# DassHydro-dev/smash

Measured on AMD Instinct MI355X. Metric: cell-timesteps/s, forward+adjoint sweep, higher is better.
Workload: dtype f32

## Files before the change

smash_amd/csrc/smashx.hip:

```cpp
#include "../../include/smashx.h"

#include <hip/hip_runtime.h>
#include <rccl/rccl.h>

#include <dlfcn.h>

#include <algorithm>
#include <functional>
#include <numeric>
#include <cstdio>
#include <cstdlib>
#include <cstring>
#include <string>
#include <vector>

#include "sx_cost.h"
#include "sx_jreg.h"
#include "sx_kernels.h"
#include "sx_ensemble.h"
#include "sx_resident.h"
#include "sx_fields.h"
#include "sx_interception.h"
#include "sx_meanforcing.h"
#include "sx_prcpindices.h"
// ... 1090 lines not shown
                        hipStream_t st, bool* ok) {
    const int h0 = p->flay.pet_hour0;
    const int d0 = (t0 + h0) / 24, d1 = (t0 + rows - 1 + h0) / 24;
    for (int r0 = 0; r0 < rows; r0 += 32768) {
        const int rr = std::min(32768, rows - r0);
        hipLaunchKernelGGL(k_encode_prcp, dim3((p->n + 255) / 256, rr), dim3(256), 0, st, p->d_prcp16 + (size_t)(t0 + r0) * p->npad,
                           d_prcp_src + (size_t)r0 * ld, idx, p->n, p->npad, ld, rr, p->flay.prcp_factor, p->d_fstatus);
    }
    hipLaunchKernelGGL(k_encode_pet, dim3((p->n + 255) / 256, d1 - d0 + 1), dim3(256), 0, st, p->d_petd, d_pet_src, idx, p->n, p->npad, ld,
                       t0, rows, h0, p->d_ratio, p->d_fstatus);
    unsigned status[2] = {0, 0};
    HIPCHK(hipMemcpyAsync(status, p->d_fstatus, sizeof(status), hipMemcpyDeviceToHost, st));
    HIPCHK(hipStreamSynchronize(st));
    HIPCHK(hipGetLastError());
    *ok = status[0] == 0;
    if (status[1]) { float g; std::memcpy(&g, &status[1], 4); p->A.prcp_gap = g; }
    p->petd_open = true;
    return 0;
}

int smashx_set_forcing_layout(smashx_plan* p, const smashx_forcing_layout* lay) {
    if (!p || !lay) return fail(SMASHX_E_ARG, "null argument");
    if (p->d_prcp || p->d_prcp16) {
        if (p->have_forcing && !p->d_prcp16 == !lay->compact) return fail(SMASHX_E_STATE, "the forcing is already resident in this layout");
        int rc = set_device(p); if (rc) return rc;
        HIPCHK(hipStreamSynchronize(p->stream)); HIPCHK(hipStreamSynchronize(p->stream_r));
        drop_compact(p);
        p->dfree(p->d_prcp); p->dfree(p->d_pet); p->d_prcp = p->d_pet = nullptr; p->A.prcp = p->A.pet = nullptr;
        p->have_forcing = false;
        p->block_seen.clear();
    }
    if (lay->compact) {
        if (p->cfg.dt != 3600.f) return fail(SMASHX_E_UNSUPPORTED, "compact forcing: the daily-PET form is defined for dt = 3600 s");
        if (!(lay->prcp_factor > 0.f) || lay->pet_hour0 < 0 || lay->pet_hour0 > 23) return fail(SMASHX_E_ARG, "bad prcp_factor / pet_hour0");
        for (int h = 0; h < 24; ++h) if (!(lay->pet_ratio[h] >= 0.f)) return fail(SMASHX_E_ARG, "pet_ratio must be >= 0");
    }
    p->flay = *lay;
    return 0;
}

int smashx_forcing_info(const smashx_plan* p, int* compact, double* bytes_per_cellstep) {
    if (!p) return fail(SMASHX_E_ARG, "null plan");
    const bool c = p->d_prcp16 != nullptr || (!p->d_prcp && p->flay.compact);
    if (compact) *compact = c ? 1 : 0;
    if (bytes_per_cellstep) *bytes_per_cellstep = c ? 2.0 + 4.0 * ((p->nt + p->flay.pet_hour0 + 23) / 24) / (double)p->nt : 8.0;
    return 0;
}

int smashx_set_forcing(smashx_plan* p, const float* prcp, const float* pet, int sparse) {
    if (!p || !prcp || !pet) return fail(SMASHX_E_ARG, "null argument");
    int rc = set_device(p); if (rc) return rc;
    if (sparse && !p->d_sparse_idx) return fail(SMASHX_E_ARG, "sparse forcing needs mesh.path at plan creation");
    const long plane = sparse ? p->n_sparse : p->n2;
    const int* idx = sparse ? p->d_sparse_idx : p->d_cell_flat;
    for (int attempt = 0; attempt < 2; ++attempt) {
        if ((rc = alloc_forcing(p))) return rc;
        const bool compact = p->d_prcp16 != nullptr;
        bool ok = true;
        if (compact) {
            const long half = std::max<long>(1, p->stage_planes / 2);
            HIPCHK(hipMemsetAsync(p->d_fstatus, 0, 2 * sizeof(unsigned), p->stream));
            HIPCHK(hipMemsetAsync(p->d_petd, 0xFF, (size_t)p->ndays * p->npad * sizeof(float), p->stream));
            for (int t = 0; t < p->nt && ok;) {
                int rows = (int)std::min<long>(half, p->nt - t);
                const int to_day_end = 24 - (t + p->flay.pet_hour0) % 24;
                if (rows > to_day_end) rows = to_day_end + (rows - to_day_end) / 24 * 24;
                float* sp = p->d_stage; float* se = p->d_stage + (size_t)half * p->n2;
                HIPCHK(hipMemcpyAsync(sp, prcp + (size_t)t * plane, (size_t)rows * plane * 4, hipMemcpyHostToDevice, p->stream));
// ... 2316 lines not shown
```

smash_amd/csrc/sx_kernels.h:

```cpp
#pragma once

#include <hip/hip_runtime.h>

#include <climits>

#include "sx_ops.h"
#include "sx_tangent.h"
#include "sx_vic.h"

#define SX_BT 4
#define SX_VBLOCK 256

__device__ __forceinline__ void sx_lds_barrier() {
    __builtin_amdgcn_fence(__ATOMIC_RELEASE, "workgroup", "local");
    __builtin_amdgcn_s_barrier();
    __builtin_amdgcn_fence(__ATOMIC_ACQUIRE, "workgroup", "local");
}

__device__ __forceinline__ void sx_lds_wave_fence() {
    __builtin_amdgcn_fence(__ATOMIC_RELEASE, "workgroup", "local");
    __builtin_amdgcn_wave_barrier();
    __builtin_amdgcn_fence(__ATOMIC_ACQUIRE, "workgroup", "local");
}

// ... 198 lines not shown
            if (i < niter && lane) {
                fifo[wpos] = v;
                const float4 o = fifo[rpos];
                wpos = wpos + 1 == depth ? 0 : wpos + 1;
                rpos = rpos + 1 == depth ? 0 : rpos + 1;
                if (GATHER) {
                    const int tb = i - d;
                    sx_gstore4(stag + (size_t)(i + smin) * A.ncs, (tb >= 0 && tb < nb) ? o : zero4);
                } else {
                    const int tb = i - spread;
                    if (plain && tb >= 0) sx_gstore4(plain + (size_t)tb * pstride, o);
                }
            }
        }
    }
}

__global__ void sx_k_prep_routing(SxDeviceArrays A) {
    SX_LIBM_INIT();
    const int k = blockIdx.x * blockDim.x + threadIdx.x;
    if (k >= A.n) return;
    const float lr = A.lr[k];
    const float f = (float)(A.flwacc[k] - 1);
    A.rt_a[k] = sx_expf(-A.dt / (lr * 60.f));
    A.rt_f[k] = f;
    A.rt_denf[k] = 0.001f * A.dx * A.dx * f;
    A.rt_denb[k] = 0.001f * (A.dx * A.dx) * f;
}

#define SX_NT 2
#ifndef SX_STILL
#define SX_STILL 1
#endif
#define SX_HIK 8
#ifndef SX_VADJ_NT
#define SX_VADJ_NT 0
#endif
template <int AUX = 0>
__device__ __forceinline__ float sx_row_load(const float* row, unsigned byte_off) {
    const __amdgpu_buffer_rsrc_t r = __builtin_amdgcn_make_buffer_rsrc((void*)row, 0, 0x7fffffff, 0x00020000);
    return __builtin_bit_cast(float, __builtin_amdgcn_raw_buffer_load_b32(r, byte_off, 0, AUX));
}
template <int AUX = 0>
__device__ __forceinline__ void sx_row_store4(float* row, unsigned byte_off, float a, float b, float c, float d) {
    typedef int sx_v4i __attribute__((ext_vector_type(4)));
    const __amdgpu_buffer_rsrc_t r = __builtin_amdgcn_make_buffer_rsrc((void*)row, 0, 0x7fffffff, 0x00020000);
    sx_v4i v = {__builtin_bit_cast(int, a), __builtin_bit_cast(int, b), __builtin_bit_cast(int, c), __builtin_bit_cast(int, d)};
    __builtin_amdgcn_raw_buffer_store_b128(v, r, byte_off, 0, AUX);
}
template <int AUX = 0>
__device__ __forceinline__ void sx_row_store(float* row, unsigned byte_off, float v) {
    const __amdgpu_buffer_rsrc_t r = __builtin_amdgcn_make_buffer_rsrc((void*)row, 0, 0x7fffffff, 0x00020000);
    __builtin_amdgcn_raw_buffer_store_b32(__builtin_bit_cast(int, v), r, byte_off, 0, AUX);
}

template <int AUX = 0>
__device__ __forceinline__ unsigned sx_row_load_u16(const unsigned short* row, unsigned byte_off) {
    const __amdgpu_buffer_rsrc_t r = __builtin_amdgcn_make_buffer_rsrc((void*)row, 0, 0x7fffffff, 0x00020000);
    return (unsigned)(unsigned short)__builtin_amdgcn_raw_buffer_load_b16(r, byte_off, 0, AUX);
}

__device__ __forceinline__ float sx_prcp_decode(const SxDeviceArrays& A, unsigned k) {
    const float v = (float)k * A.prcp_c;
    return k == 65535u ? A.prcp_gap : v;
}

typedef const __attribute__((address_space(4))) float sx_cfloat;
template <bool COMPACT>
struct SxForcing {
    const SxDeviceArrays& A;
    const unsigned kb;
    const size_t npad;
    int h;
    const char* prow; const char* erow;
    unsigned p_n, p_w; float e_n, e_w, r_n, r_w;
    __device__ __forceinline__ SxForcing(const SxDeviceArrays& A_, unsigned kb_, int t_first)
        : A(A_), kb(kb_), npad((size_t)A_.npad), h(COMPACT ? (t_first + A_.hour0) % 24 : 0),
          prow(COMPACT ? (const char*)(A_.prcp16 + (size_t)t_first * A_.npad) : (const char*)(A_.prcp + (size_t)t_first * A_.npad)),
          erow(COMPACT ? nullptr : (const char*)(A_.pet + (size_t)t_first * A_.npad)),
          p_n(0u), p_w(0u), e_n(0.f), e_w(0.f), r_n(0.f), r_w(0.f) {}
    template <int AUX, bool BACK> __device__ __forceinline__ void request(int t, bool first) {
        const long step = (long)npad * (COMPACT ? 2 : 4) * (BACK ? -1 : 1);
        if (!COMPACT) {
            p_n = __float_as_uint(sx_row_load<AUX>((const float*)prow, kb));
            e_n = sx_row_load<AUX>((const float*)erow, kb);
            prow += step; erow += step;
            return;
        }
        p_n = __float_as_uint(sx_row_load<AUX>((const float*)prow, (kb >> 1) & ~3u));
        prow += step;
        if (first || h == (BACK ? 23 : 0)) e_n = sx_row_load<AUX>(A.petd + (size_t)((t + A.hour0) / 24) * npad, kb);
        r_n = sx_row_load(A.pet_ratio + h, 0u);
        h = BACK ? (h == 0 ? 23 : h - 1) : (h == 23 ? 0 : h + 1);
    }
    __device__ __forceinline__ void hold() {
        p_w = p_n; e_w = e_n; r_w = r_n;
        sx_pinu(p_w); sx_pin1(e_w);
        if (COMPACT) sx_pin1(r_w);
    }
    __device__ __forceinline__ float prcp() const {
        if (!COMPACT) return __uint_as_float(p_w);
        return sx_prcp_decode(A, (p_w >> ((kb & 4u) << 2)) & 0xffffu);
    }
    __device__ __forceinline__ float pet() const {
        if (!COMPACT) return e_w;
        return e_w < 0.f ? e_w : e_w * r_w;
    }
};

template <bool ROW = true, class Cell>
__device__ __forceinline__ void sx_forcing_at(const SxDeviceArrays& A, int t, Cell c, float& p, float& e) {
    const size_t npad = (size_t)A.npad;
    if (A.prcp16 == nullptr) {
        if (ROW) { p = sx_row_load(A.prcp + (size_t)t * npad, c); e = sx_row_load(A.pet + (size_t)t * npad, c); }
        else { p = A.prcp[(size_t)t * npad + c]; e = A.pet[(size_t)t * npad + c]; }
        return;
    }
    p = sx_prcp_decode(A, ROW ? sx_row_load_u16(A.prcp16 + (size_t)t * npad, c >> 1) : (unsigned)A.prcp16[(size_t)t * npad + c]);
    const int q = t + A.hour0;
    const float D = ROW ? sx_row_load(A.petd + (size_t)(q / 24) * npad, c) : A.petd[(size_t)(q / 24) * npad + c];
    e = D < 0.f ? D : D * (ROW ? ((sx_cfloat*)A.pet_ratio)[q % 24] : A.pet_ratio[q % 24]);
}

#ifndef SX_VFWD_WAVES
#define SX_VFWD_WAVES 8
#endif
template <int ST, bool TAPE, bool CF>
#ifndef SX_VFWD_WAVES_GRC
#define SX_VFWD_WAVES_GRC 7
#endif
__global__ __launch_bounds__(SX_VBLOCK, (ST == 2 && CF) ? SX_VFWD_WAVES : (ST == 3 && TAPE && CF) ? SX_VFWD_WAVES_GRC : 1)
void sx_k_vert_fwd(SxDeviceArrays A, int t0, int T) {
    SX_LIBM_INIT();
    const int k = A.k0 + blockIdx.x * SX_VBLOCK + threadIdx.x;
    if (k >= A.k1) return;
    const size_t npad = (size_t)A.npad;

    const SxPlanCell<> cell{A, k};
    SxCellParams P;
    float hi = 0.f, hp = 0.f, hft = 0.f, hst = 0.f;
    sx_cell_params<ST>(cell, P);
    sx_fwd_powers<ST>(P);
    sx_levels_in<ST>(cell, hi, hp, hft, hst);

    const unsigned kb = (unsigned)k * 4u;
    SxForcing<CF> F(A, kb, t0);
    if (T > 0) F.template request<SX_NT, false>(t0, true);
    for (int tq = 0; tq * 4 < T; ++tq) {
        float q[4] = {0.f, 0.f, 0.f, 0.f};
#pragma unroll
        for (int i = 0; i < 4; ++i) {
            const int tt = tq * 4 + i;
            if (tt < T) {
                F.hold();
                if (tt + 1 < T) F.template request<SX_NT, false>(t0 + tt + 1, false);
                const float prcp = F.prcp(), pet = F.pet();
                if (TAPE) {
                    const size_t o = (size_t)tt * npad;
                    if (ST == 2 || ST == 3) {
                        if (A.tape_hi) sx_row_store<SX_NT>(A.tape_hi + o, kb, hi);
                        else if ((tt % SX_HIK) == 0) sx_row_store<SX_NT>(A.ckpt_hi + (size_t)(tt / SX_HIK) * npad, kb, hi);
                    }
                    sx_row_store<SX_NT>(A.tape_hp + o, kb, hp);
                    sx_row_store<SX_NT>(A.tape_hft + o, kb, hft);
                    if (ST == 3) sx_row_store<SX_NT>(A.tape_hst + o, kb, hst);
                }
                const bool still = SX_STILL && sx_wave_all(sx_is_still<ST>(prcp, pet, hi, hp));
                q[i] = sx_vertical_step<ST>(P, prcp, pet, hi, hp, hft, hst, still);
            }
        }
        sx_row_store4<SX_NT>(A.qtT + (size_t)tq * npad * 4, kb * 4u, q[0], q[1], q[2], q[3]);
    }
    sx_levels_out<ST>(cell, hi, hp, hft, hst);
}

__device__ __forceinline__ SxVicParams sx_vic_load(const SxDeviceArrays& A, int k) {
    return sx_vic_params(SxPlanCell<>{A, k});
}
#ifndef SX_VFWD_WAVES_VIC
#define SX_VFWD_WAVES_VIC 5
#endif
template <bool TAPE, bool CF>
__global__ __launch_bounds__(SX_VBLOCK, TAPE ? SX_VFWD_WAVES_VIC : 1) void sx_k_vert_fwd_vic(SxDeviceArrays A, int t0, int T) {
    SX_LIBM_INIT();
    const int k = A.k0 + blockIdx.x * SX_VBLOCK + threadIdx.x;
    if (k >= A.k1) return;
    const size_t npad = (size_t)A.npad;
    const SxVicParams P = sx_vic_load(A, k);
    const float cusl2_m4 = sx_pow_m4(P.cusl2);
    float husl1 = A.hi[k], husl2 = A.hp[k], hlsl = A.hft[k];
    const unsigned kb = (unsigned)k * 4u;
    SxForcing<CF> F(A, kb, t0);
    if (T > 0) F.template request<SX_NT, false>(t0, true);
    for (int tq = 0; tq * 4 < T; ++tq) {
        float q[4] = {0.f, 0.f, 0.f, 0.f};
#pragma unroll
        for (int i = 0; i < 4; ++i) {
            const int tt = tq * 4 + i;
            if (tt < T) {
                F.hold();
                if (tt + 1 < T) F.template request<SX_NT, false>(t0 + tt + 1, false);
                if (TAPE) {
                    const size_t o = (size_t)tt * npad;
                    sx_row_store<SX_NT>(A.tape_hi + o, kb, husl1);
                    sx_row_store<SX_NT>(A.tape_hp + o, kb, husl2);
                    sx_row_store<SX_NT>(A.tape_hft + o, kb, hlsl);
                }
                q[i] = sx_vic_step(P, cusl2_m4, F.prcp(), F.pet(), husl1, husl2, hlsl);
            }
        }
        sx_row_store4<SX_NT>(A.qtT + (size_t)tq * npad * 4, kb * 4u, q[0], q[1], q[2], q[3]);
    }
    A.hi[k] = husl1; A.hp[k] = husl2; A.hft[k] = hlsl;
}

#ifndef SX_VADJ_WAVES_VIC
#define SX_VADJ_WAVES_VIC 3
#endif
template <bool CF>
__global__ __launch_bounds__(SX_VBLOCK, SX_VADJ_WAVES_VIC) void sx_k_vert_adj_vic(SxDeviceArrays A, int t0, int T) {
    SX_LIBM_INIT();
    const int k = A.k0 + blockIdx.x * SX_VBLOCK + threadIdx.x;
    if (k >= A.k1) return;
    const size_t npad = (size_t)A.npad;
    const SxVicParams P = sx_vic_load(A, k);
    float cusl2_m4, cusl2_m5;
    sx_pow_m4_m5(P.cusl2, &cusl2_m4, &cusl2_m5);
    const SxPlanCell<true> grad{A, k};
    SxVicGrads G;
    sx_vic_fields_in(grad, G.b_b, G.cusl1_b, G.cusl2_b, G.clsl_b, G.ks_b, G.ds_b, G.dsm_b, G.ws_b);
    sx_vic_levels_in(grad, G.husl1_b, G.husl2_b, G.hlsl_b);
    const unsigned kb = (unsigned)k * 4u;
    SxForcing<CF> F(A, kb, t0 + T - 1);
    float n_h1 = 0.f, n_h2 = 0.f, n_hl = 0.f, n_q = 0.f;
    auto fetch = [&](int tt, bool first) {
        const size_t o = (size_t)tt * npad;
        F.template request<SX_VADJ_NT, true>(t0 + tt, first);
        n_h1 = sx_row_load<SX_VADJ_NT>(A.tape_hi + o, kb); n_h2 = sx_row_load<SX_VADJ_NT>(A.tape_hp + o, kb);
        n_hl = sx_row_load<SX_VADJ_NT>(A.tape_hft + o, kb);
        n_q = sx_row_load(A.qtT + (size_t)(tt >> 2) * npad * 4 + (tt & 3), kb * 4u);
    };
    if (T > 0) fetch(T - 1, true);
    for (int tt = T - 1; tt >= 0; --tt) {
        float h1 = n_h1, h2 = n_h2, hl = n_hl, q_b = n_q;
        F.hold();
        sx_pin1(h1); sx_pin1(h2); sx_pin1(hl); sx_pin1(q_b);
        if (tt > 0) fetch(tt - 1, false);
        sx_vic_step_b(P, cusl2_m4, cusl2_m5, F.prcp(), F.pet(), h1, h2, hl, q_b, G);
    }
    sx_vic_fields_out(grad, G.b_b, G.cusl1_b, G.cusl2_b, G.clsl_b, G.ks_b, G.ds_b, G.dsm_b, G.ws_b);
    sx_vic_levels_out(grad, G.husl1_b, G.husl2_b, G.hlsl_b);
}

__global__ __launch_bounds__(SX_VBLOCK) void sx_k_vert_fwd_vic_d(SxDeviceArrays A, int t0, int T) {
    SX_LIBM_INIT();
    const int k = A.k0 + blockIdx.x * SX_VBLOCK + threadIdx.x;
    if (k >= A.k1) return;
    const size_t npad = (size_t)A.npad;
    const SxVicParams P = sx_vic_load(A, k);
    SxVicTan D;
    sx_vic_fields_in(SxPlanCell<true>{A, k}, D.b_d, D.cusl1_d, D.cusl2_d, D.clsl_d, D.ks_d, D.ds_d, D.dsm_d, D.ws_d);
    float cusl2_m4, cusl2_m5;
    sx_pow_m4_m5(P.cusl2, &cusl2_m4, &cusl2_m5);
    SxVD husl1 = sx_vd(A.hi[k], A.hi_b[k]), husl2 = sx_vd(A.hp[k], A.hp_b[k]), hlsl = sx_vd(A.hft[k], A.hft_b[k]);
    float* qt = A.qtT + (size_t)k * 4;
    float* qd = A.qtdT + (size_t)k * 4;
    for (int tt = 0; tt < T; ++tt) {
        float prcp, pet;
        sx_forcing_at(A, t0 + tt, (unsigned)k * 4u, prcp, pet);
        const SxVD r = sx_vic_step_d(P, D, cusl2_m4, cusl2_m5, prcp, pet, husl1, husl2, hlsl);
        const size_t o = (size_t)(tt >> 2) * npad * 4 + (tt & 3);
        qt[o] = r.v; qd[o] = r.d;
    }
    A.hi[k] = husl1.v; A.hi_b[k] = husl1.d; A.hp[k] = husl2.v; A.hp_b[k] = husl2.d; A.hft[k] = hlsl.v; A.hft_b[k] = hlsl.d;
}

template <int ST>
__global__ __launch_bounds__(SX_VBLOCK) void sx_k_vert_fwd_d(SxDeviceArrays A, int t0, int T) {
    SX_LIBM_INIT();
    const int k = A.k0 + blockIdx.x * SX_VBLOCK + threadIdx.x;
    if (k >= A.k1) return;
// ... 475 lines not shown
#ifndef SX_VADJ_WAVES
#define SX_VADJ_WAVES 5
#endif
template <int ST, bool CF>
#ifndef SX_VADJ_WAVES_GRC
#if SX_EXACT_LIBM
#define SX_VADJ_WAVES_GRC 1
#else
#define SX_VADJ_WAVES_GRC 5
#endif
#endif
__global__ __launch_bounds__(SX_VBLOCK, (ST == 2 && CF) ? SX_VADJ_WAVES : (ST == 3 && CF) ? SX_VADJ_WAVES_GRC : 1)
void sx_k_vert_adj(SxDeviceArrays A, int t0, int T) {
    SX_LIBM_INIT();
    const int k = A.k0 + blockIdx.x * SX_VBLOCK + threadIdx.x;
    if (k >= A.k1) return;
    const size_t npad = (size_t)A.npad;
    SxCellParams P;
    sx_cell_params<ST>(SxPlanCell<>{A, k}, P);
    SxAdjParams Q;
    sx_adj_params<ST>(P, Q);
    SxCellGrads G;
    G.ci_b = (ST == 2 || ST == 3) ? A.ci_b[k] : 0.f;
    G.cp_b = A.cp_b[k];
    G.cft_b = A.cft_b[k];
    G.cst_b = (ST == 3) ? A.cst_b[k] : 0.f;
    G.exc_b = (ST != 4) ? A.exc_b[k] : 0.f;
    G.hi_b = (ST == 2 || ST == 3) ? A.hi_b[k] : 0.f;
    G.hp_b = A.hp_b[k];
    G.hft_b = A.hft_b[k];
    G.hst_b = (ST == 3) ? A.hst_b[k] : 0.f;
    const unsigned kb = (unsigned)k * 4u;
    SxForcing<CF> F(A, kb, t0 + T - 1);
    float n_hi = 0.f, n_hp = 0.f, n_hft = 0.f, n_hst = 0.f, n_q = 0.f;
    const bool hi_taped = (ST == 2 || ST == 3) && A.tape_hi != nullptr;
    const size_t olast = (size_t)(T > 0 ? T - 1 : 0) * npad;
    const float* r_hi = hi_taped ? A.tape_hi + olast : nullptr;
    const float* r_hp = A.tape_hp + olast;
    const float* r_hft = A.tape_hft + olast;
    const float* r_hst = (ST == 3) ? A.tape_hst + olast : nullptr;
    auto fetch = [&](int tt, bool first) {
        F.template request<SX_VADJ_NT, true>(t0 + tt, first);
        if (hi_taped) { n_hi = sx_row_load<SX_VADJ_NT>(r_hi, kb); r_hi -= npad; }
        n_hp = sx_row_load<SX_VADJ_NT>(r_hp, kb); n_hft = sx_row_load<SX_VADJ_NT>(r_hft, kb);
        r_hp -= npad; r_hft -= npad;
        if (ST == 3) { n_hst = sx_row_load<SX_VADJ_NT>(r_hst, kb); r_hst -= npad; }
        n_q = sx_row_load(A.qtT + (size_t)(tt >> 2) * npad * 4 + (tt & 3), kb * 4u);
    };
    __shared__ float s_hi[(ST == 2 || ST == 3) ? SX_HIK : 1][SX_VBLOCK];
    if (T > 0) fetch(T - 1, true);
    for (int tb = (T - 1) / SX_HIK; tb >= 0; --tb) {
        const int tt0 = tb * SX_HIK, len = min(SX_HIK, T - tt0);
        if ((ST == 2 || ST == 3) && !hi_taped) {
            float fp[SX_HIK], fe[SX_HIK];
#pragma unroll
            for (int j = 0; j < SX_HIK; ++j) sx_forcing_at(A, t0 + tt0 + (j < len ? j : 0), kb, fp[j], fe[j]);
            float h = sx_row_load(A.ckpt_hi + (size_t)tb * npad, kb);
#pragma unroll
            for (int j = 0; j < SX_HIK; ++j) {
                s_hi[j][threadIdx.x] = h;
                if (j < len && fp[j] >= 0.f && fe[j] >= 0.f) { float pn, ei; sx_interception(fp[j], fe[j], P.ci, P.dci, h, pn, ei); }
            }
        }
        for (int tt = tt0 + len - 1; tt >= tt0; --tt) {
            float hit = n_hi, hp = n_hp, hft = n_hft, hst = n_hst, q = n_q;
            F.hold();
            sx_pin1(hp); sx_pin1(hft); sx_pin1(q);
            if (ST == 2 || ST == 3) sx_pin1(hit);
            if (ST == 3) sx_pin1(hst);
            if (tt > 0) fetch(tt - 1, false);
            const float prcp = F.prcp(), pet = F.pet();
            const float hi = (ST == 2 || ST == 3) ? (hi_taped ? hit : s_hi[tt - tt0][threadIdx.x]) : 0.f;
            const bool still = SX_STILL && sx_wave_all(sx_is_still<ST>(prcp, pet, hi, hp));
            sx_vertical_step_b<ST>(P, Q, prcp, pet, hi, hp, hft, hst, q, G, still);
        }
    }
    if (ST == 2 || ST == 3) { A.ci_b[k] = G.ci_b; A.hi_b[k] = G.hi_b; }
    A.cp_b[k] = G.cp_b;
    A.cft_b[k] = G.cft_b;
    if (ST == 3) { A.cst_b[k] = G.cst_b; A.hst_b[k] = G.hst_b; }
    if (ST != 4) A.exc_b[k] = G.exc_b;
    A.hp_b[k] = G.hp_b;
    A.hft_b[k] = G.hft_b;
}
```

smash_amd/csrc/sx_ops.h:

```cpp
#pragma once

#include "sx_fields.h"
#include "sx_math.h"

#define SX_DEV __device__ __forceinline__

SX_DEV bool sx_wave_all(bool pred) { return __builtin_amdgcn_ballot_w64(!pred) == 0ull; }
SX_DEV bool sx_wave_any(bool pred) { return __builtin_amdgcn_ballot_w64(pred) != 0ull; }

struct SxCellParams {
    float ci, cp, inv_cp, cft, cst, exc;
    float cft_m4, cst_m4;
    SxDiv dci, dcft, dcst;
};

SX_DEV void sx_cell_params_init(SxCellParams& P) {
    P.inv_cp = 1.f / P.cp;
    P.dci = sx_mkdiv(P.ci);
    P.dcft = sx_mkdiv(P.cft);
    P.dcst = sx_mkdiv(P.cst);
}

template <int ST, class Src>
SX_DEV void sx_cell_params(const Src& src, SxCellParams& P) {
// ... 122 lines not shown
        if (ST == 1 || ST == 4) {
            ei = fminf(pet, prcp);
            pn = fmaxf(0.f, prcp - ei);
        } else {
            sx_interception(prcp, pet, P.ci, P.dci, hi, pn, ei);
        }
        en = pet - ei;
        sx_production(pn, en, P.cp, P.inv_cp, hp, pr, perc);
        if (ST != 4) l = P.exc * sx_pow_3p5(hft);
    }
    float qr, ql, qd, qt;
    if (ST == 1 || ST == 2) {
        const float prr = 0.9f * (pr + perc) + l;
        const float prd = 0.1f * (pr + perc);
        sx_transfer(prcp, prr, P.cft, P.dcft, P.cft_m4, hft, qr);
        qd = fmaxf(0.f, prd + l);
        qt = (qr + qd);
    } else if (ST == 3) {
        const float prr = 0.9f * 0.6f * (pr + perc) + l;
        const float prl = 0.9f * 0.4f * (pr + perc);
        const float prd = 0.1f * (pr + perc);
        sx_transfer(prcp, prr, P.cft, P.dcft, P.cft_m4, hft, qr);
        sx_transfer(prcp, prl, P.cst, P.dcst, P.cst_m4, hst, ql);
        qd = fmaxf(0.f, prd + l);
        qt = (qr + ql + qd);
    } else {
        const float prr = pr + perc;
        sx_transfer(prcp, prr, P.cft, P.dcft, P.cft_m4, hft, qr);
        qt = qr;
    }
    return qt;
}

template <int ST>
SX_DEV bool sx_is_still(float prcp, float pet, float hi, float hp) {
    bool s = (prcp == 0.f) & (pet == 0.f) & (fabsf(hp) < 15.f);
    if (ST == 2 || ST == 3) s = s & (hi >= 0.f) & (hi <= 1.f);
    return s | !(prcp >= 0.f && pet >= 0.f);
}

SX_DEV void sx_interception_b(float prcp, float pet, float ci, const SxDiv& dci, float& ci_b, float hi, float& hi_b, float& pn_b, float& ei_b) {
    float ei, pn;
    bool br_ei, br_pn;
    if (pet > prcp + hi * ci) { ei = prcp + hi * ci; br_ei = true; } else { ei = pet; br_ei = false; }
    if (0.f < prcp - ci * (1.f - hi) - ei) { pn = prcp - ci * (1.f - hi) - ei; br_pn = true; } else { pn = 0.f; br_pn = false; }
    const float temp_b = sx_div(hi_b, dci);
    ei_b = ei_b - temp_b;
    pn_b = pn_b - temp_b;
    ci_b = ci_b - sx_div((prcp - ei - pn) * temp_b, dci);
    if (br_pn) {
        ci_b = ci_b - (1.f - hi) * pn_b;
        hi_b = hi_b + ci * pn_b;
        ei_b = ei_b - pn_b;
    }
    if (br_ei) {
        hi_b = hi_b + ci * ei_b;
        ci_b = ci_b + hi * ei_b;
    }
}

SX_DEV void sx_production_b(const SxProd& R, float pn, float& pn_b, float en, float& en_b, float cp, float inv_cp,
                            const SxDiv& dcp2, float& cp_b, float hp, float& hp_b, float pr_b, float perc_b) {
    const SxDiv db4 = {1.0e12f, 1.0f / 1.0e12f};
    const float thp = R.thp, the = R.the, ps = R.ps, es = R.es, hp_imd = R.hp_imd, pwr1 = R.pwr1, perc = R.perc;
    perc_b = perc_b - inv_cp * hp_b;
    float inv_cp_b = -(perc * hp_b);
    cp_b = cp_b + hp_imd * (1.f - pwr1) * perc_b;
    const float pwr1_b = -(hp_imd * cp * perc_b);
    const float pwx1_b = -(0.25f * R.pw125 * pwr1_b);
    float hp_imd_b = hp_b + cp * (1.f - pwr1) * perc_b + sx_div(4.f * (hp_imd * hp_imd * hp_imd) * pwx1_b, db4);
// ... 31 lines not shown
        temp_b4 = temp0 * es_b;
        temp_b5 = 0.f;
        hp_b = hp_b + hp_imd_b;
        en_b = inv_cp * temp_b4;
    }
    float temp_b2;
    const float temp2 = cp * (-(hp * hp) + 1.f);
    if (wp) {
        if (wp) {
            const float temp = thp, temp1 = thp;
            const SxDiv d0 = sx_mkdiv_fast(hp * temp + 1.f);
            temp_b = sx_div(ps_b, d0);
            temp_b0 = (1.0f - thp * thp) * temp2 * temp_b;
            const float temp_b1 = -sx_div(temp2 * temp1 * temp_b, d0);
            hp_b = hp_b + temp * temp_b1 - 2.f * hp * cp * temp1 * temp_b;
            temp_b2 = (1.0f - thp * thp) * hp * temp_b1;
            inv_cp_b = inv_cp_b + (ps - es) * hp_imd_b + en * temp_b5 + en * temp_b4 + pn * temp_b2 + pn * temp_b0;
            cp_b = cp_b + (1.f - hp * hp) * temp1 * temp_b - sx_div(inv_cp_b, dcp2);
        } else {
            temp_b0 = temp2 * ps_b;
            temp_b2 = 0.f;
            inv_cp_b = inv_cp_b + (ps - es) * hp_imd_b + en * temp_b5 + en * temp_b4;
            cp_b = cp_b - sx_div(inv_cp_b, dcp2);
        }
    } else {
        temp_b0 = temp2 * ps_b;
        temp_b2 = 0.f;
        inv_cp_b = inv_cp_b + (ps - es) * hp_imd_b + en * temp_b5 + en * temp_b4;
        cp_b = cp_b - sx_div(inv_cp_b, dcp2);
    }
    pn_b = pn_b + inv_cp * temp_b2 + inv_cp * temp_b0;
}

SX_DEV void sx_transfer_b(float prcp, float pr, float& pr_b, float ct, const SxDiv& dct, const SxDiv& dct2, float ct_m4,
                          float ct_m5, float& ct_b, float ht, float& ht_b, float q_b) {
    float pr_imd = pr, g_pwx1 = 0.f, g_pwx3 = 0.f;
    const bool gap = prcp < 0.f;
    const bool any_gap = gap;
    if (any_gap) {
        if (gap) {
            g_pwx1 = ht * ct;
            g_pwx3 = sx_pow_m4(g_pwx1) - ct_m4;
            pr_imd = sx_pow_m025(g_pwx3) - ht * ct;
        }
    }
    const float ht_try = ht + sx_div(pr_imd, dct);
    const bool br_max = 1.e-6f < ht_try;
    const float ht_imd = br_max ? ht_try : 1.e-6f;
    const float pwx1 = ht_imd * ct;
    float pwr1, pwx1_m5;
    sx_pow_m4_m5(pwx1, &pwr1, &pwx1_m5);
    const float pwx3 = pwr1 + ct_m4;
    float pwr3, pwx3_m125;
    sx_pow_m025_m125(pwx3, &pwr3, &pwx3_m125);
    const float ht_new = sx_div(pwr3, dct);
    float htb = ht_b - ct * q_b;
    float pwr3_b = sx_div(htb, dct);
    float pwx3_b = -0.25f * pwx3_m125 * pwr3_b;
    float pwr1_b = pwx3_b, pwr2_b = pwx3_b;
    float pwx1_b = -4.f * pwx1_m5 * pwr1_b;
    const float ht_imd_b = ct * q_b + ct * pwx1_b;
    ct_b = ct_b + (ht_imd - ht_new) * q_b + -4.f * ct_m5 * pwr2_b - sx_div(pwr3 * htb, dct2) + ht_imd * pwx1_b;
    const float pr_imd_b1 = sx_div(ht_imd_b, dct), ct_b1 = ct_b - sx_div(pr_imd * ht_imd_b, dct2);
    htb = br_max ? ht_imd_b : 0.f;
    const float pr_imd_b = br_max ? pr_imd_b1 : 0.f;
    ct_b = br_max ? ct_b1 : ct_b;
    pr_b = gap ? 0.f : pr_imd_b;
    if (any_gap) {
        if (gap) {
            pwr3_b = pr_imd_b;
// ... 1 lines not shown
            if (g_pwx3 > 0.f) sx_pow_m025_m125(g_pwx3, &g_m025, &g_m125);
            sx_pow_m4_m5(g_pwx1, &g_m4, &g_m5);
            pwx3_b = (g_pwx3 <= 0.f) ? 0.f : -0.25f * g_m125 * pwr3_b;
            pwr1_b = pwx3_b;
            pwr2_b = -pwx3_b;
            pwx1_b = -4.f * g_m5 * pwr1_b;
            htb = htb + ct * pwx1_b - ct * pr_imd_b;
            ct_b = ct_b + -4.f * ct_m5 * pwr2_b - ht * pr_imd_b + ht * pwx1_b;
        }
    }
    ht_b = htb;
}

struct SxCellGrads {
    float ci_b, cp_b, cft_b, cst_b, exc_b;
    float hi_b, hp_b, hft_b, hst_b;
};

struct SxAdjParams {
    float cft_m5, cst_m5;
    SxDiv dcft2, dcst2, dcp2;
};
template <int ST>
SX_DEV void sx_adj_params(SxCellParams& P, SxAdjParams& Q) {
    Q.cst_m5 = 1.f;
    sx_pow_m4_m5(P.cft, &P.cft_m4, &Q.cft_m5);
    P.cst_m4 = 1.f;
    if (ST == 3) sx_pow_m4_m5(P.cst, &P.cst_m4, &Q.cst_m5);
    Q.dcft2 = sx_mkdiv(P.cft * P.cft);
    Q.dcst2 = sx_mkdiv(P.cst * P.cst);
    Q.dcp2 = sx_mkdiv(P.cp * P.cp);
}

template <int ST>
SX_DEV void sx_vertical_step_b(const SxCellParams& P, const SxAdjParams& Q, float prcp, float pet, float hi, float hp,
                               float hft, float hst, float qt_b, SxCellGrads& G, bool still = false) {
    const bool wet = prcp >= 0.f && pet >= 0.f;
    float ei = 0.f, pn = 0.f, en = 0.f, pr = 0.f, perc = 0.f, l = 0.f, prr, prl = 0.f, prd = 0.f;
    float h35 = 0.f, h25 = 0.f;
    SxProd R;
    if (wet) {
        if (!still) {
            float hi2 = hi;
            if (ST == 1 || ST == 4) { ei = fminf(pet, prcp); pn = fmaxf(0.f, prcp - ei); }
            else sx_interception(prcp, pet, P.ci, P.dci, hi2, pn, ei);
            en = pet - ei;
            R = sx_production_full<true>(pn, en, P.cp, P.inv_cp, hp);
            pr = R.pr; perc = R.perc;
        }
        if (ST != 4) { sx_pow_3p5_2p5(hft, &h35, &h25); l = P.exc * h35; }
    }
    if (ST == 1 || ST == 2) { prr = 0.9f * (pr + perc) + l; prd = 0.1f * (pr + perc); }
    else if (ST == 3) { prr = 0.9f * 0.6f * (pr + perc) + l; prl = 0.9f * 0.4f * (pr + perc); prd = 0.1f * (pr + perc); }
    else prr = pr + perc;

    const float qr_b = qt_b, ql_b = qt_b, qd_b = qt_b;
    float prd_b = 0.f, l_b = 0.f, prr_b = 0.f, prl_b = 0.f, pr_b, perc_b;
    if (ST != 4) {
        if (0.f < prd + l) { prd_b = qd_b; l_b = qd_b; }
    }
    if (ST == 3) sx_transfer_b(prcp, prl, prl_b, P.cst, P.dcst, Q.dcst2, P.cst_m4, Q.cst_m5, G.cst_b, hst, G.hst_b, ql_b);
    sx_transfer_b(prcp, prr, prr_b, P.cft, P.dcft, Q.dcft2, P.cft_m4, Q.cft_m5, G.cft_b, hft, G.hft_b, qr_b);
    if (ST == 1 || ST == 2) {
        pr_b = 0.1f * prd_b + 0.9f * prr_b;
        perc_b = 0.1f * prd_b + 0.9f * prr_b;
        l_b = l_b + prr_b;
    } else if (ST == 3) {
        float tb = 0.4f * 0.9f * prl_b;
        pr_b = 0.1f * prd_b + tb;
        perc_b = 0.1f * prd_b + tb;
        tb = 0.6f * 0.9f * prr_b;
        l_b = l_b + prr_b;
        pr_b = pr_b + tb;
        perc_b = perc_b + tb;
    } else {
        pr_b = prr_b;
        perc_b = prr_b;
    }
    if (wet) {
        float pn_b = 0.f, en_b = 0.f;
        if (ST != 4) {
            G.exc_b = G.exc_b + h35 * l_b;
            G.hft_b = G.hft_b + 3.5f * h25 * P.exc * l_b;
        }
        if (still) {
            const SxDiv db4 = {1.0e12f, 1.0f / 1.0e12f};
            const float hp_imd = hp + 0.f;
            perc_b = perc_b - P.inv_cp * G.hp_b;
            const float pwr1_b = -(hp_imd * P.cp * perc_b);
            const float pwx1_b = -(0.25f * pwr1_b);
            G.hp_b = 0.f + (G.hp_b + (P.cp * 0.f) * perc_b + sx_div(4.f * (hp_imd * hp_imd * hp_imd) * pwx1_b, db4));
            return;
        }
        sx_production_b(R, pn, pn_b, en, en_b, P.cp, P.inv_cp, Q.dcp2, G.cp_b, hp, G.hp_b, pr_b, perc_b);
        if (ST == 2 || ST == 3) {
// ... 6 lines not shown
```

Baseline: 57.64 billion.

## Double-buffer forcing registers and add wave-uniform gap-free adjoint fast path

Forcing and tape prefetch values are kept in two alternating register slots, selected by compile-time parity, instead of being copied from a 'next' slot into a 'working' slot each step. This removes register moves and gives the scheduler more freedom in the forward and adjoint vertical loops. In the adjoint for structure 2, when every lane of the wave has valid (non-gap) forcing, a specialised step is taken that drops the gap checks and gap-handling branches. The validation of compact forcing also now rejects infinite factors. The risks are more register pressure from the doubled buffers and extra code size from the duplicated specialised adjoint step.

New measurement: 58.32 billion (median of 6 runs). 1.01x the previous value.

```diff
diff --git a/smash_amd/csrc/smashx.hip b/smash_amd/csrc/smashx.hip
--- a/smash_amd/csrc/smashx.hip
+++ b/smash_amd/csrc/smashx.hip
@@ -1146,8 +1146,8 @@
     }
     if (lay->compact) {
         if (p->cfg.dt != 3600.f) return fail(SMASHX_E_UNSUPPORTED, "compact forcing: the daily-PET form is defined for dt = 3600 s");
-        if (!(lay->prcp_factor > 0.f) || lay->pet_hour0 < 0 || lay->pet_hour0 > 23) return fail(SMASHX_E_ARG, "bad prcp_factor / pet_hour0");
-        for (int h = 0; h < 24; ++h) if (!(lay->pet_ratio[h] >= 0.f)) return fail(SMASHX_E_ARG, "pet_ratio must be >= 0");
+        if (!(lay->prcp_factor > 0.f) || __builtin_isinf(lay->prcp_factor) || lay->pet_hour0 < 0 || lay->pet_hour0 > 23) return fail(SMASHX_E_ARG, "bad prcp_factor / pet_hour0");
+        for (int h = 0; h < 24; ++h) if (!(lay->pet_ratio[h] >= 0.f) || __builtin_isinf(lay->pet_ratio[h])) return fail(SMASHX_E_ARG, "pet_ratio must be >= 0 and finite");
     }
     p->flay = *lay;
     return 0;
diff --git a/smash_amd/csrc/sx_kernels.h b/smash_amd/csrc/sx_kernels.h
--- a/smash_amd/csrc/sx_kernels.h
+++ b/smash_amd/csrc/sx_kernels.h
@@ -254,6 +254,9 @@
 #ifndef SX_STILL
 #define SX_STILL 1
 #endif
+#ifndef SX_GAPFREE
+#define SX_GAPFREE 1
+#endif
 #define SX_HIK 8
 #ifndef SX_VADJ_NT
 #define SX_VADJ_NT 0
@@ -288,6 +291,7 @@
 }
 
 typedef const __attribute__((address_space(4))) float sx_cfloat;
+template <int S> struct SxSet { static constexpr int value = S; };
 template <bool COMPACT>
 struct SxForcing {
     const SxDeviceArrays& A;
@@ -295,38 +299,49 @@
     const size_t npad;
     int h;
     const char* prow; const char* erow;
-    unsigned p_n, p_w; float e_n, e_w, r_n, r_w;
+    unsigned p_[2]; float e_[2], r_[2];
     __device__ __forceinline__ SxForcing(const SxDeviceArrays& A_, unsigned kb_, int t_first)
         : A(A_), kb(kb_), npad((size_t)A_.npad), h(COMPACT ? (t_first + A_.hour0) % 24 : 0),
           prow(COMPACT ? (const char*)(A_.prcp16 + (size_t)t_first * A_.npad) : (const char*)(A_.prcp + (size_t)t_first * A_.npad)),
           erow(COMPACT ? nullptr : (const char*)(A_.pet + (size_t)t_first * A_.npad)),
-          p_n(0u), p_w(0u), e_n(0.f), e_w(0.f), r_n(0.f), r_w(0.f) {}
-    template <int AUX, bool BACK> __device__ __forceinline__ void request(int t, bool first) {
+          p_{0u, 0u}, e_{0.f, 0.f}, r_{0.f, 0.f} {}
+    template <int AUX, bool BACK, int S, bool HANDED = true> __device__ __forceinline__ void request(int t, bool first) {
         const long step = (long)npad * (COMPACT ? 2 : 4) * (BACK ? -1 : 1);
         if (!COMPACT) {
-            p_n = __float_as_uint(sx_row_load<AUX>((const float*)prow, kb));
-            e_n = sx_row_load<AUX>((const float*)erow, kb);
+            p_[S] = __float_as_uint(sx_row_load<AUX>((const float*)prow, kb));
+            e_[S] = sx_row_load<AUX>((const float*)erow, kb);
             prow += step; erow += step;
             return;
         }
-        p_n = __float_as_uint(sx_row_load<AUX>((const float*)prow, (kb >> 1) & ~3u));
+        p_[S] = __float_as_uint(sx_row_load<AUX>((const float*)prow, (kb >> 1) & ~3u));
         prow += step;
-        if (first || h == (BACK ? 23 : 0)) e_n = sx_row_load<AUX>(A.petd + (size_t)((t + A.hour0) / 24) * npad, kb);
-        r_n = sx_row_load(A.pet_ratio + h, 0u);
+        if (first || h == (BACK ? 23 : 0)) e_[S] = sx_row_load<AUX>(A.petd + (size_t)((t + A.hour0) / 24) * npad, kb);
+        else if (HANDED) e_[S] = e_[1 - S];
+        r_[S] = sx_row_load(A.pet_ratio + h, 0u);
         h = BACK ? (h == 0 ? 23 : h - 1) : (h == 23 ? 0 : h + 1);
     }
-    __device__ __forceinline__ void hold() {
-        p_w = p_n; e_w = e_n; r_w = r_n;
-        sx_pinu(p_w); sx_pin1(e_w);
-        if (COMPACT) sx_pin1(r_w);
-    }
-    __device__ __forceinline__ float prcp() const {
-        if (!COMPACT) return __uint_as_float(p_w);
-        return sx_prcp_decode(A, (p_w >> ((kb & 4u) << 2)) & 0xffffu);
-    }
-    __device__ __forceinline__ float pet() const {
-        if (!COMPACT) return e_w;
-        return e_w < 0.f ? e_w : e_w * r_w;
+    template <int S> __device__ __forceinline__ void hold() {
+        sx_pinu(p_[S]); sx_pin1(e_[S]);
+        if (COMPACT) sx_pin1(r_[S]);
+    }
+    __device__ __forceinline__ void hold_copy() {
+        p_[0] = p_[1]; e_[0] = e_[1]; r_[0] = r_[1];
+        hold<0>();
+    }
+    template <int S> __device__ __forceinline__ unsigned count() const { return (p_[S] >> ((kb & 4u) << 2)) & 0xffffu; }
+    template <int S> __device__ __forceinline__ bool no_gap() const {
+        if (!COMPACT) return __uint_as_float(p_[S]) >= 0.f && e_[S] >= 0.f;
+        return count<S>() != 65535u && __builtin_amdgcn_classf(e_[S], 0x1e0);
+    }
+    template <int S, bool NOGAP = false> __device__ __forceinline__ float prcp() const {
+        if (!COMPACT) return __uint_as_float(p_[S]);
+        if (NOGAP) return (float)count<S>() * A.prcp_c;
+        return sx_prcp_decode(A, count<S>());
+    }
+    template <int S, bool NOGAP = false> __device__ __forceinline__ float pet() const {
+        if (!COMPACT) return e_[S];
+        if (NOGAP) return e_[S] * r_[S];
+        return e_[S] < 0.f ? e_[S] : e_[S] * r_[S];
     }
 };
 
@@ -367,33 +382,37 @@
 
     const unsigned kb = (unsigned)k * 4u;
     SxForcing<CF> F(A, kb, t0);
-    if (T > 0) F.template request<SX_NT, false>(t0, true);
+    auto step = [&](auto S, int tt) -> float {
+        constexpr int s = decltype(S)::value;
+        F.template hold<s>();
+        if (tt + 1 < T) F.template request<SX_NT, false, 1 - s>(t0 + tt + 1, false);
+        if (TAPE) {
+            const size_t o = (size_t)tt * npad;
+            if (ST == 2 || ST == 3) {
+                if (A.tape_hi) sx_row_store<SX_NT>(A.tape_hi + o, kb, hi);
+                else if ((tt % SX_HIK) == 0) sx_row_store<SX_NT>(A.ckpt_hi + (size_t)(tt / SX_HIK) * npad, kb, hi);
+            }
+            sx_row_store<SX_NT>(A.tape_hp + o, kb, hp);
+            sx_row_store<SX_NT>(A.tape_hft + o, kb, hft);
+            if (ST == 3) sx_row_store<SX_NT>(A.tape_hst + o, kb, hst);
+        }
+        const float prcp = F.template prcp<s>(), pet = F.template pet<s>();
+        const bool still = SX_STILL && sx_wave_all(sx_is_still<ST>(prcp, pet, hi, hp));
+        return sx_vertical_step<ST>(P, prcp, pet, hi, hp, hft, hst, still);
+    };
+    if (T > 0) F.template request<SX_NT, false, 0>(t0, true);
     for (int tq = 0; tq * 4 < T; ++tq) {
         float q[4] = {0.f, 0.f, 0.f, 0.f};
 #pragma unroll
         for (int i = 0; i < 4; ++i) {
             const int tt = tq * 4 + i;
-            if (tt < T) {
-                F.hold();
-                if (tt + 1 < T) F.template request<SX_NT, false>(t0 + tt + 1, false);
-                const float prcp = F.prcp(), pet = F.pet();
-                if (TAPE) {
-                    const size_t o = (size_t)tt * npad;
-                    if (ST == 2 || ST == 3) {
-                        if (A.tape_hi) sx_row_store<SX_NT>(A.tape_hi + o, kb, hi);
-                        else if ((tt % SX_HIK) == 0) sx_row_store<SX_NT>(A.ckpt_hi + (size_t)(tt / SX_HIK) * npad, kb, hi);
-                    }
-                    sx_row_store<SX_NT>(A.tape_hp + o, kb, hp);
-                    sx_row_store<SX_NT>(A.tape_hft + o, kb, hft);
-                    if (ST == 3) sx_row_store<SX_NT>(A.tape_hst + o, kb, hst);
-                }
-                const bool still = SX_STILL && sx_wave_all(sx_is_still<ST>(prcp, pet, hi, hp));
-                q[i] = sx_vertical_step<ST>(P, prcp, pet, hi, hp, hft, hst, still);
-            }
+            if (tt < T) q[i] = (i & 1) ? step(SxSet<1>{}, tt) : step(SxSet<0>{}, tt);
         }
         sx_row_store4<SX_NT>(A.qtT + (size_t)tq * npad * 4, kb * 4u, q[0], q[1], q[2], q[3]);
     }
-    sx_levels_out<ST>(cell, hi, hp, hft, hst);
+    unsigned ke = (unsigned)k;
+    sx_pinu(ke);
+    sx_levels_out<ST>(SxPlanCell<>{A, (int)ke}, hi, hp, hft, hst);
 }
 
 __device__ __forceinline__ SxVicParams sx_vic_load(const SxDeviceArrays& A, int k) {
@@ -413,22 +432,22 @@
     float husl1 = A.hi[k], husl2 = A.hp[k], hlsl = A.hft[k];
     const unsigned kb = (unsigned)k * 4u;
     SxForcing<CF> F(A, kb, t0);
-    if (T > 0) F.template request<SX_NT, false>(t0, true);
+    if (T > 0) F.template request<SX_NT, false, 1, false>(t0, true);
     for (int tq = 0; tq * 4 < T; ++tq) {
         float q[4] = {0.f, 0.f, 0.f, 0.f};
 #pragma unroll
         for (int i = 0; i < 4; ++i) {
             const int tt = tq * 4 + i;
             if (tt < T) {
-                F.hold();
-                if (tt + 1 < T) F.template request<SX_NT, false>(t0 + tt + 1, false);
+                F.hold_copy();
+                if (tt + 1 < T) F.template request<SX_NT, false, 1, false>(t0 + tt + 1, false);
                 if (TAPE) {
                     const size_t o = (size_t)tt * npad;
                     sx_row_store<SX_NT>(A.tape_hi + o, kb, husl1);
                     sx_row_store<SX_NT>(A.tape_hp + o, kb, husl2);
                     sx_row_store<SX_NT>(A.tape_hft + o, kb, hlsl);
                 }
-                q[i] = sx_vic_step(P, cusl2_m4, F.prcp(), F.pet(), husl1, husl2, hlsl);
+                q[i] = sx_vic_step(P, cusl2_m4, F.template prcp<0>(), F.template pet<0>(), husl1, husl2, hlsl);
             }
         }
         sx_row_store4<SX_NT>(A.qtT + (size_t)tq * npad * 4, kb * 4u, q[0], q[1], q[2], q[3]);
@@ -457,7 +476,7 @@
     float n_h1 = 0.f, n_h2 = 0.f, n_hl = 0.f, n_q = 0.f;
     auto fetch = [&](int tt, bool first) {
         const size_t o = (size_t)tt * npad;
-        F.template request<SX_VADJ_NT, true>(t0 + tt, first);
+        F.template request<SX_VADJ_NT, true, 1, false>(t0 + tt, first);
         n_h1 = sx_row_load<SX_VADJ_NT>(A.tape_hi + o, kb); n_h2 = sx_row_load<SX_VADJ_NT>(A.tape_hp + o, kb);
         n_hl = sx_row_load<SX_VADJ_NT>(A.tape_hft + o, kb);
         n_q = sx_row_load(A.qtT + (size_t)(tt >> 2) * npad * 4 + (tt & 3), kb * 4u);
@@ -465,10 +484,10 @@
     if (T > 0) fetch(T - 1, true);
     for (int tt = T - 1; tt >= 0; --tt) {
         float h1 = n_h1, h2 = n_h2, hl = n_hl, q_b = n_q;
-        F.hold();
+        F.hold_copy();
         sx_pin1(h1); sx_pin1(h2); sx_pin1(hl); sx_pin1(q_b);
         if (tt > 0) fetch(tt - 1, false);
-        sx_vic_step_b(P, cusl2_m4, cusl2_m5, F.prcp(), F.pet(), h1, h2, hl, q_b, G);
+        sx_vic_step_b(P, cusl2_m4, cusl2_m5, F.template prcp<0>(), F.template pet<0>(), h1, h2, hl, q_b, G);
     }
     sx_vic_fields_out(grad, G.b_b, G.cusl1_b, G.cusl2_b, G.clsl_b, G.ks_b, G.ds_b, G.dsm_b, G.ws_b);
     sx_vic_levels_out(grad, G.husl1_b, G.husl2_b, G.hlsl_b);
@@ -1010,23 +1029,43 @@
     G.hst_b = (ST == 3) ? A.hst_b[k] : 0.f;
     const unsigned kb = (unsigned)k * 4u;
     SxForcing<CF> F(A, kb, t0 + T - 1);
-    float n_hi = 0.f, n_hp = 0.f, n_hft = 0.f, n_hst = 0.f, n_q = 0.f;
+    float n_hi[2] = {0.f, 0.f}, n_hp[2] = {0.f, 0.f}, n_hft[2] = {0.f, 0.f}, n_hst[2] = {0.f, 0.f}, n_q[2] = {0.f, 0.f};
     const bool hi_taped = (ST == 2 || ST == 3) && A.tape_hi != nullptr;
     const size_t olast = (size_t)(T > 0 ? T - 1 : 0) * npad;
     const float* r_hi = hi_taped ? A.tape_hi + olast : nullptr;
     const float* r_hp = A.tape_hp + olast;
     const float* r_hft = A.tape_hft + olast;
     const float* r_hst = (ST == 3) ? A.tape_hst + olast : nullptr;
-    auto fetch = [&](int tt, bool first) {
-        F.template request<SX_VADJ_NT, true>(t0 + tt, first);
-        if (hi_taped) { n_hi = sx_row_load<SX_VADJ_NT>(r_hi, kb); r_hi -= npad; }
-        n_hp = sx_row_load<SX_VADJ_NT>(r_hp, kb); n_hft = sx_row_load<SX_VADJ_NT>(r_hft, kb);
+    auto fetch = [&](auto S, int tt, bool first) {
+        constexpr int s = decltype(S)::value;
+        F.template request<SX_VADJ_NT, true, s>(t0 + tt, first);
+        if (hi_taped) { n_hi[s] = sx_row_load<SX_VADJ_NT>(r_hi, kb); r_hi -= npad; }
+        n_hp[s] = sx_row_load<SX_VADJ_NT>(r_hp, kb); n_hft[s] = sx_row_load<SX_VADJ_NT>(r_hft, kb);
         r_hp -= npad; r_hft -= npad;
-        if (ST == 3) { n_hst = sx_row_load<SX_VADJ_NT>(r_hst, kb); r_hst -= npad; }
-        n_q = sx_row_load(A.qtT + (size_t)(tt >> 2) * npad * 4 + (tt & 3), kb * 4u);
+        if (ST == 3) { n_hst[s] = sx_row_load<SX_VADJ_NT>(r_hst, kb); r_hst -= npad; }
+        n_q[s] = sx_row_load(A.qtT + (size_t)(tt >> 2) * npad * 4 + (tt & 3), kb * 4u);
     };
     __shared__ float s_hi[(ST == 2 || ST == 3) ? SX_HIK : 1][SX_VBLOCK];
-    if (T > 0) fetch(T - 1, true);
+    auto step = [&](auto S, int tt, int tt0) {
+        constexpr int s = decltype(S)::value;
+        __builtin_amdgcn_sched_barrier(0);
+        F.template hold<s>();
+        sx_pin1(n_hp[s]); sx_pin1(n_hft[s]); sx_pin1(n_q[s]);
+        if (ST == 2 || ST == 3) sx_pin1(n_hi[s]);
+        if (ST == 3) sx_pin1(n_hst[s]);
+        if (tt > 0) fetch(SxSet<1 - s>{}, tt - 1, false);
+        const float hi = (ST == 2 || ST == 3) ? (hi_taped ? n_hi[s] : s_hi[tt - tt0][threadIdx.x]) : 0.f;
+        if (SX_GAPFREE && ST == 2 && sx_wave_all(F.template no_gap<s>())) {
+            const float prcp = F.template prcp<s, true>(), pet = F.template pet<s, true>();
+            const bool still = SX_STILL && sx_wave_all(sx_is_still<ST, true>(prcp, pet, hi, n_hp[s]));
+            sx_vertical_step_b<ST, true>(P, Q, prcp, pet, hi, n_hp[s], n_hft[s], n_hst[s], n_q[s], G, still);
+            return;
+        }
+        const float prcp = F.template prcp<s>(), pet = F.template pet<s>();
+        const bool still = SX_STILL && sx_wave_all(sx_is_still<ST>(prcp, pet, hi, n_hp[s]));
+        sx_vertical_step_b<ST>(P, Q, prcp, pet, hi, n_hp[s], n_hft[s], n_hst[s], n_q[s], G, still);
+    };
+    if (T > 0) { if ((T - 1) & 1) fetch(SxSet<1>{}, T - 1, true); else fetch(SxSet<0>{}, T - 1, true); }
     for (int tb = (T - 1) / SX_HIK; tb >= 0; --tb) {
         const int tt0 = tb * SX_HIK, len = min(SX_HIK, T - tt0);
         if ((ST == 2 || ST == 3) && !hi_taped) {
@@ -1040,24 +1079,21 @@
                 if (j < len && fp[j] >= 0.f && fe[j] >= 0.f) { float pn, ei; sx_interception(fp[j], fe[j], P.ci, P.dci, h, pn, ei); }
             }
         }
-        for (int tt = tt0 + len - 1; tt >= tt0; --tt) {
-            float hit = n_hi, hp = n_hp, hft = n_hft, hst = n_hst, q = n_q;
-            F.hold();
-            sx_pin1(hp); sx_pin1(hft); sx_pin1(q);
-            if (ST == 2 || ST == 3) sx_pin1(hit);
-            if (ST == 3) sx_pin1(hst);
-            if (tt > 0) fetch(tt - 1, false);
-            const float prcp = F.prcp(), pet = F.pet();
-            const float hi = (ST == 2 || ST == 3) ? (hi_taped ? hit : s_hi[tt - tt0][threadIdx.x]) : 0.f;
-            const bool still = SX_STILL && sx_wave_all(sx_is_still<ST>(prcp, pet, hi, hp));
-            sx_vertical_step_b<ST>(P, Q, prcp, pet, hi, hp, hft, hst, q, G, still);
-        }
-    }
-    if (ST == 2 || ST == 3) { A.ci_b[k] = G.ci_b; A.hi_b[k] = G.hi_b; }
-    A.cp_b[k] = G.cp_b;
-    A.cft_b[k] = G.cft_b;
-    if (ST == 3) { A.cst_b[k] = G.cst_b; A.hst_b[k] = G.hst_b; }
-    if (ST != 4) A.exc_b[k] = G.exc_b;
-    A.hp_b[k] = G.hp_b;
-    A.hft_b[k] = G.hft_b;
-}
+        int tt = tt0 + len - 1;
+        bool odd = (tt & 1) != 0;
+        while (tt >= tt0) {
+            if (odd) { step(SxSet<1>{}, tt, tt0); --tt; }
+            step(SxSet<0>{}, tt, tt0); --tt;
+            odd = true;
+        }
+    }
+    unsigned ke = (unsigned)k;
+    sx_pinu(ke);
+    if (ST == 2 || ST == 3) { A.ci_b[ke] = G.ci_b; A.hi_b[ke] = G.hi_b; }
+    A.cp_b[ke] = G.cp_b;
+    A.cft_b[ke] = G.cft_b;
+    if (ST == 3) { A.cst_b[ke] = G.cst_b; A.hst_b[ke] = G.hst_b; }
+    if (ST != 4) A.exc_b[ke] = G.exc_b;
+    A.hp_b[ke] = G.hp_b;
+    A.hft_b[ke] = G.hft_b;
+}
diff --git a/smash_amd/csrc/sx_ops.h b/smash_amd/csrc/sx_ops.h
--- a/smash_amd/csrc/sx_ops.h
+++ b/smash_amd/csrc/sx_ops.h
@@ -178,10 +178,11 @@
     return qt;
 }
 
-template <int ST>
+template <int ST, bool NOGAP = false>
 SX_DEV bool sx_is_still(float prcp, float pet, float hi, float hp) {
     bool s = (prcp == 0.f) & (pet == 0.f) & (fabsf(hp) < 15.f);
     if (ST == 2 || ST == 3) s = s & (hi >= 0.f) & (hi <= 1.f);
+    if (NOGAP) return s;
     return s | !(prcp >= 0.f && pet >= 0.f);
 }
 
@@ -279,10 +280,11 @@
     pn_b = pn_b + inv_cp * temp_b2 + inv_cp * temp_b0;
 }
 
+template <bool NOGAP = false>
 SX_DEV void sx_transfer_b(float prcp, float pr, float& pr_b, float ct, const SxDiv& dct, const SxDiv& dct2, float ct_m4,
                           float ct_m5, float& ct_b, float ht, float& ht_b, float q_b) {
     float pr_imd = pr, g_pwx1 = 0.f, g_pwx3 = 0.f;
-    const bool gap = prcp < 0.f;
+    const bool gap = !NOGAP && prcp < 0.f;
     const bool any_gap = gap;
     if (any_gap) {
         if (gap) {
@@ -350,10 +352,10 @@
     Q.dcp2 = sx_mkdiv(P.cp * P.cp);
 }
 
-template <int ST>
+template <int ST, bool NOGAP = false>
 SX_DEV void sx_vertical_step_b(const SxCellParams& P, const SxAdjParams& Q, float prcp, float pet, float hi, float hp,
                                float hft, float hst, float qt_b, SxCellGrads& G, bool still = false) {
-    const bool wet = prcp >= 0.f && pet >= 0.f;
+    const bool wet = NOGAP || (prcp >= 0.f && pet >= 0.f);
     float ei = 0.f, pn = 0.f, en = 0.f, pr = 0.f, perc = 0.f, l = 0.f, prr, prl = 0.f, prd = 0.f;
     float h35 = 0.f, h25 = 0.f;
     SxProd R;
@@ -377,8 +379,8 @@
     if (ST != 4) {
         if (0.f < prd + l) { prd_b = qd_b; l_b = qd_b; }
     }
-    if (ST == 3) sx_transfer_b(prcp, prl, prl_b, P.cst, P.dcst, Q.dcst2, P.cst_m4, Q.cst_m5, G.cst_b, hst, G.hst_b, ql_b);
-    sx_transfer_b(prcp, prr, prr_b, P.cft, P.dcft, Q.dcft2, P.cft_m4, Q.cft_m5, G.cft_b, hft, G.hft_b, qr_b);
+    if (ST == 3) sx_transfer_b<NOGAP>(prcp, prl, prl_b, P.cst, P.dcst, Q.dcst2, P.cst_m4, Q.cst_m5, G.cst_b, hst, G.hst_b, ql_b);
+    sx_transfer_b<NOGAP>(prcp, prr, prr_b, P.cft, P.dcft, Q.dcft2, P.cft_m4, Q.cft_m5, G.cft_b, hft, G.hft_b, qr_b);
     if (ST == 1 || ST == 2) {
         pr_b = 0.1f * prd_b + 0.9f * prr_b;
         perc_b = 0.1f * prd_b + 0.9f * prr_b;
```
